# gau-nernst/llama-x

Hardware: AMD Instinct MI355X
Metric: train tokens/sec Llama-3.1-8B seq4096 at 1/2/4/8 MI355X; p50 step ms (higher is better)
Workload: dtype bf16; 1 GPU; Llama-3.1-8B text-only LoRA r=16 bf16, seq=4096, 1 sequence per GPU, causal mask, base+LM head frozen (BASELINE.json configs[1]); random-init weights at 8B dimensions; seq_len=4096, parallelism=dp1, launch=hipGraph replay (fwd+bwd+AdamW), lm_head_rows=labelled only

## Files before the change

llama-x_amd/csrc/attn_bwd.hip:

```cpp
#include "attn.h"
#include "attn_dropout.h"

typedef __attribute__((ext_vector_type(8))) short s16x8_t;

__device__ __forceinline__ int dual_swz(int row) { return ((row & 3) << 2) | ((row >> 2) & 3); }
__device__ __forceinline__ uint32_t dual_swz(uint32_t row) { return ((row & 3) << 2) | ((row >> 2) & 3); }

__device__ __forceinline__ bf16x8_t tr_frag(const char* img, int row0, int db, int lane) {
  const int hh = lane >> 5, tq = (lane & 15) >> 2, tp = lane & 3, tsub = (lane >> 4) & 1;
  const int chunk = 4 * db + 2 * tsub + (tp >> 1);
  const int rlo = row0 + 4 * hh + tq, rhi = rlo + 8;
  s16x4_t lo = __builtin_amdgcn_ds_read_tr16_b64_v4i16((lds_s16x4*)(img + rlo * 256 + ((chunk ^ dual_swz(rlo)) << 4) + ((tp & 1) << 3)));
  s16x4_t hi = __builtin_amdgcn_ds_read_tr16_b64_v4i16((lds_s16x4*)(img + rhi * 256 + ((chunk ^ dual_swz(rhi)) << 4) + ((tp & 1) << 3)));
  s16x8_t v = {lo[0], lo[1], lo[2], lo[3], hi[0], hi[1], hi[2], hi[3]};
  return __builtin_bit_cast(bf16x8_t, v);
}

__device__ __forceinline__ bf16x8_t row_frag(const char* img, int row, int ks, int hh) {
  return *reinterpret_cast<const bf16x8_t*>(img + row * 256 + (((2 * ks + hh) ^ dual_swz(row)) << 4));
}

template <int N>
__device__ __forceinline__ void lds_tr_wait(s16x4_t& a, s16x4_t& b, s16x4_t (&c)[4], s16x4_t (&d)[4]) {
  asm volatile("s_waitcnt lgkmcnt(%10)"
               : "+v"(a), "+v"(b), "+v"(c[0]), "+v"(c[1]), "+v"(c[2]), "+v"(c[3]), "+v"(d[0]), "+v"(d[1]), "+v"(d[2]), "+v"(d[3])
               : "n"(N));
  __builtin_amdgcn_sched_barrier(0);
}
__device__ __forceinline__ uint32_t xor_imm(uint32_t a, int c) {
  if (c == 0) return a;
  uint32_t r;
  asm volatile("v_xor_b32 %0, %1, %2" : "=v"(r) : "n"(c), "v"(a));
  return r;
}

struct AttnBwdArgs {
  const bf16_t* q; const bf16_t* k; const bf16_t* v; const bf16_t* o; const bf16_t* d_o;
  const float* lse; float* delta; float* nlse;
  const float* rope;
  unsigned long long* stamps;
  bf16_t* dq; bf16_t* dk; bf16_t* dv;
  bf16_t* ds; int Sp;
  int64_t q_sb, q_ss, k_sb, k_ss, v_sb, v_ss, o_sb, o_ss, do_sb, do_ss;
  int64_t dq_sb, dq_ss, dk_sb, dk_ss, dv_sb, dv_ss;
  const int* doc_ids; const int* prefix_len; const uint8_t* flags;
  int B, S, H, KVH;
  float scale, scale_log2;
  const uint8_t* mask; int64_t m_sb, m_sq;
  const int64_t* rng; uint32_t drop_thr; float drop_c; int stream_id;
};

enum { BWD_CAUSAL = 0, BWD_RULE = 1, BWD_MASK = 2 };

__device__ __forceinline__ uint32_t mask_nibble(uint32_t w) {
  const uint32_t nz = (((w & 0x7f7f7f7fu) + 0x7f7f7f7fu) | w) & 0x80808080u;
  return ((nz >> 7) * 0x01020408u) >> 24;
}

#define DQ_STAGE_BYTES (2 * TILE_BYTES)
#define DQ_LDS_BYTES (2 * DQ_STAGE_BYTES)

template <int MODE, bool DROPOUT = false>
__global__ __launch_bounds__(256, 2) void attn_bwd_dq_kernel(const AttnBwdArgs a) {
  static_assert(!(DROPOUT && MODE == BWD_MASK), "dropout exists in the causal and the rule mode");
  constexpr bool GENERAL = MODE == BWD_RULE;
  constexpr bool FLAGS = MODE != BWD_CAUSAL;
  constexpr bool MASK = MODE == BWD_MASK;
  extern __shared__ __attribute__((aligned(256))) char smem[];
  const int tid = threadIdx.x, lane = tid & 63;
  const int wave = __builtin_amdgcn_readfirstlane(tid >> 6);
  const int nqb = (a.S + BQ - 1) / BQ, nkt = (a.S + BKV - 1) / BKV;
  const int qb = nqb - 1 - blockIdx.y;
  const int h = blockIdx.x, b = blockIdx.z;
  const int kvh = h / (a.H / a.KVH);
  const int r = lane & 31, hh = lane >> 5;
  const int qi = qb * BQ + wave * 32 + r;
  const int qrow = min(qi, a.S - 1);

  const uint8_t* fl = FLAGS ? a.flags + ((int64_t)b * nqb + qb) * nkt : nullptr;
  const int kt_end = FLAGS ? nkt : min(nkt, (qb * BQ + BQ + BKV - 1) / BKV);
  uint32_t fpack = 0;
  int fchunk = -1;
  auto tile_class = [&](int t) -> int {
    if constexpr (FLAGS) {
      if ((t >> 6) != fchunk) {
        fchunk = t >> 6;
        fpack = fl[min(fchunk * 64 + lane, nkt - 1)];
      }
      return __builtin_amdgcn_readlane((int)fpack, t & 63);
    } else {
      return (t * BKV + BKV - 1 <= qb * BQ) ? 2 : 1;
    }
  };
  auto next_tile = [&](int t) {
    while (t < kt_end && tile_class(t) == 0) ++t;
    return t;
  };

  const int srow_in = lane >> 4, sslot = lane & 15;
  const bf16_t* kbase = a.k + (int64_t)b * a.k_sb + kvh * HD;
  const bf16_t* vbase = a.v + (int64_t)b * a.v_sb + kvh * HD;
  uint32_t koff[4], voff[4];
#pragma unroll
  for (int i = 0; i < 4; ++i) {
    const int row = i * 16 + wave * 4 + srow_in;
    koff[i] = (uint32_t)(((int64_t)row * a.k_ss + (sslot ^ dual_swz(row)) * 8) * 2);
    voff[i] = (uint32_t)(((int64_t)row * a.v_ss + (sslot ^ (row & 15)) * 8) * 2);
  }
  auto stage = [&](int buf, int t) {
    char* sK = smem + buf * DQ_STAGE_BYTES;
    char* sV = sK + TILE_BYTES;
    if (t * BKV + BKV <= a.S) {
      const char* kt = (const char*)(kbase + (int64_t)t * BKV * a.k_ss);
      const char* vt = (const char*)(vbase + (int64_t)t * BKV * a.v_ss);
      if constexpr (DROPOUT) {
        uint32_t l0;
        asm volatile("v_mbcnt_lo_u32_b32 %0, -1, 0\n\tv_mbcnt_hi_u32_b32 %0, -1, %0" : "=v"(l0));
        const int slot = (int)(l0 & 15);
#pragma unroll
        for (int i = 0; i < 4; ++i) {
          const int row = i * 16 + wave * 4 + (int)(l0 >> 4);
          const uint32_t ko = (uint32_t)(((int64_t)row * a.k_ss + (slot ^ dual_swz(row)) * 8) * 2);
          const uint32_t vo = (uint32_t)(((int64_t)row * a.v_ss + (slot ^ (row & 15)) * 8) * 2);
          __builtin_amdgcn_global_load_lds((gbl_void*)(kt + ko), (lds_void*)(sK + (i * 16 + wave * 4) * 256), 16, 0, 0);
          __builtin_amdgcn_global_load_lds((gbl_void*)(vt + vo), (lds_void*)(sV + (i * 16 + wave * 4) * 256), 16, 0, 0);
        }
      } else {
#pragma unroll
      for (int i = 0; i < 4; ++i) {
        __builtin_amdgcn_global_load_lds((gbl_void*)(kt + koff[i]), (lds_void*)(sK + (i * 16 + wave * 4) * 256), 16, 0, 0);
        __builtin_amdgcn_global_load_lds((gbl_void*)(vt + voff[i]), (lds_void*)(sV + (i * 16 + wave * 4) * 256), 16, 0, 0);
      }
      }
    } else {
#pragma unroll
      for (int i = 0; i < 4; ++i) {
        const int row = i * 16 + wave * 4 + srow_in;
        const int key = min(t * BKV + row, a.S - 1);
        const int kc = sslot ^ dual_swz(row);
        const int vc = sslot ^ (row & 15);
        __builtin_amdgcn_global_load_lds((gbl_void*)(kbase + (int64_t)key * a.k_ss + kc * 8), (lds_void*)(sK + (i * 16 + wave * 4) * 256), 16, 0, 0);
        __builtin_amdgcn_global_load_lds((gbl_void*)(vbase + (int64_t)key * a.v_ss + vc * 8), (lds_void*)(sV + (i * 16 + wave * 4) * 256), 16, 0, 0);
      }
// ... 15 lines not shown
  const int* docrow = (GENERAL && a.doc_ids) ? a.doc_ids + (int64_t)b * a.S : nullptr;
  const int my_doc = docrow ? docrow[qrow] : 0;
  const int my_prefix = (GENERAL && a.prefix_len) ? a.prefix_len[b] : 0;
  uint32_t mwn[MASK ? 8 : 1];
  auto mask_request = [&](int t_) {
    if constexpr (MASK) {
      uint32_t l0;
      asm volatile("v_mbcnt_lo_u32_b32 %0, -1, 0\n\tv_mbcnt_hi_u32_b32 %0, -1, %0" : "=v"(l0));
      const int hh = (int)(l0 >> 5);
      const uint8_t* mrow = a.mask + (int64_t)b * a.m_sb + (int64_t)min(qb * BQ + wave * 32 + (int)(l0 & 31), a.S - 1) * a.m_sq;
      if (t_ * BKV + BKV <= a.S) {
        const uint8_t* p = mrow + t_ * BKV + 4 * hh;
#pragma unroll
        for (int g = 0; g < 8; ++g) __builtin_memcpy(&mwn[g], p + (g >> 2) * 32 + 8 * (g & 3), 4);
      } else {
#pragma unroll
        for (int g = 0; g < 8; ++g) {
          const int g0 = t_ * BKV + (g >> 2) * 32 + 8 * (g & 3) + 4 * hh;
          __builtin_memcpy(&mwn[g], mrow + min(g0, a.S - 4), 4);
        }
      }
    }
  };
  auto mask_bits = [&](int t_) -> uint32_t {
    uint32_t bits = 0;
    if constexpr (MASK) {
      const bool ragged = t_ * BKV + BKV > a.S;
#pragma unroll
      for (int g = 0; g < 8; ++g) {
        uint32_t w = mwn[g];
        if (ragged) {
          const int g0 = t_ * BKV + (g >> 2) * 32 + 8 * (g & 3) + 4 * hh;
          const int sh = g0 - min(g0, a.S - 4);
          w = sh >= 4 ? 0u : w >> (8 * sh);
        }
        bits |= mask_nibble(w) << (4 * g);
      }
    }
    return bits;
  };

  int t = next_tile(0);
  if constexpr (MASK) {
#pragma unroll
    for (int g = 0; g < 8; ++g) mwn[g] = 0;
    if (t < kt_end && tile_class(t) == 1) mask_request(t);
  }
  if (t < kt_end) stage(0, t);
  bf16x8_t qf[8], dof[8], ovf[8];
  const float my_lse = a.lse[((int64_t)b * a.H + h) * a.S + qrow];
  {
    const bf16_t* qp = a.q + (int64_t)b * a.q_sb + (int64_t)qrow * a.q_ss + h * HD + 8 * hh;
    const bf16_t* dp = a.d_o + (int64_t)b * a.do_sb + (int64_t)qrow * a.do_ss + h * HD + 8 * hh;
    const bf16_t* op = a.o + (int64_t)b * a.o_sb + (int64_t)qrow * a.o_ss + h * HD + 8 * hh;
#pragma unroll
    for (int ks = 0; ks < 8; ++ks) {
      ovf[ks] = *reinterpret_cast<const bf16x8_t*>(op + 16 * ks);
      dof[ks] = *reinterpret_cast<const bf16x8_t*>(dp + 16 * ks);
      qf[ks] = *reinterpret_cast<const bf16x8_t*>(qp + 16 * ks);
    }
    __builtin_amdgcn_sched_barrier(0);
  }
  const float lse_safe = (my_lse == -INFINITY) ? 0.f : my_lse;
  float my_delta = 0.f;
  {
#pragma unroll
    for (int ks = 0; ks < 8; ++ks) {
#pragma unroll
      for (int j = 0; j < 8; ++j) my_delta += (float)ovf[ks][j] * (float)dof[ks][j];
    }
    my_delta += __shfl_xor(my_delta, 32, 64);
    if (hh == 0 && qi < a.S) {
      a.delta[((int64_t)b * a.H + h) * a.S + qi] = my_delta;
      a.nlse[((int64_t)b * a.H + h) * a.S + qi] = -lse_safe;
    }
  }

  asm volatile("s_waitcnt vmcnt(0)" ::: "memory");
  __syncthreads();
  int cur = 0;
  int docv = (GENERAL && docrow && t < kt_end) ? docrow[min(t * BKV + lane, a.S - 1)] : 0, docv_next = 0;
  AttnDropKey dkey = {0u, 0u};
  if constexpr (DROPOUT) dkey = attn_dropout_key(a.rng[0], a.rng[1], a.stream_id, b, h);
  while (t < kt_end) {
    int cls_m = 0;
    uint32_t mbits = 0;
    if constexpr (MASK) {
      cls_m = tile_class(t);
      if (cls_m == 1) mbits = mask_bits(t);
    }
    const int tn = next_tile(t + 1);
    if (tn < kt_end) stage(cur ^ 1, tn);
    if (GENERAL && docrow && tn < kt_end) docv_next = docrow[min(tn * BKV + lane, a.S - 1)];
    if constexpr (MASK) {
      if (tn < kt_end && tile_class(tn) == 1) mask_request(tn);
    }
    const char* sK = smem + cur * DQ_STAGE_BYTES;
    const char* sV = sK + TILE_BYTES;
    const int cls = MASK ? cls_m : tile_class(t);
#pragma unroll
    for (int kb = 0; kb < 2; ++kb) {
      f32x16_t st, dp;
      const f32x16_t zero = {0.f, 0.f, 0.f, 0.f, 0.f, 0.f, 0.f, 0.f, 0.f, 0.f, 0.f, 0.f, 0.f, 0.f, 0.f, 0.f};
      const int row = kb * 32 + r;
#pragma unroll
      for (int ks = 0; ks < 8; ++ks) {
        bf16x8_t kf = row_frag(sK, row, ks, hh);
        st = __builtin_amdgcn_mfma_f32_32x32x16_bf16(kf, qf[ks], ks == 0 ? zero : st, 0, 0, 0);
      }
      if (cls != 2) {
#pragma unroll
        for (int e = 0; e < 16; ++e) {
          if constexpr (MASK) {
            st[e] = ((mbits >> (kb * 16 + e)) & 1u) ? st[e] : -INFINITY;
          } else {
          const int kk = t * BKV + kb * 32 + (e & 3) + 8 * (e >> 2) + 4 * hh;
          bool ok = (kk < a.S) && (kk <= qi || kk < my_prefix);
          if constexpr (GENERAL) {
            const int kd = docrow ? __builtin_amdgcn_ds_bpermute((kk - t * BKV) << 2, docv) : my_doc;
            ok = ok && (kd == my_doc);
          }
          st[e] = ok ? st[e] : -INFINITY;
          }
        }
      }
#pragma unroll
      for (int e = 0; e < 16; ++e) st[e] = __builtin_amdgcn_exp2f(__builtin_fmaf(st[e], a.scale_log2, -lse_safe));
#pragma unroll
      for (int ks = 0; ks < 8; ++ks) {
        bf16x8_t vf = *reinterpret_cast<const bf16x8_t*>(sV + row * 256 + (((2 * ks + hh) ^ (row & 15)) << 4));
        dp = __builtin_amdgcn_mfma_f32_32x32x16_bf16(vf, dof[ks], ks == 0 ? zero : dp, 0, 0, 0);
      }
#pragma unroll
      for (int e = 0; e < 16; ++e) {
        float dpe = dp[e];
        if constexpr (DROPOUT) {
          const int kk = t * BKV + kb * 32 + (e & 3) + 8 * (e >> 2) + 4 * hh;
          dpe = attn_drop_keep(attn_drop_row(dkey, qi), attn_drop_col(dkey, kk), a.drop_thr) ? dpe * a.drop_c : 0.f;
        }
        st[e] = st[e] * (dpe - my_delta);
      }
      {
        const uint32_t kb_ = sbase + cur * DQ_STAGE_BYTES + kb * 8192 + aK0;
        s16x4_t Kl[4], Kh[4];
#pragma unroll
        for (int s = 0; s < 2; ++s) {
#pragma unroll
          for (int db = 0; db < 4; ++db) {
            if (s == 0) { lds_tr_read<0>(Kl[db], xor_imm(kb_, db << 6)); lds_tr_read<2048>(Kh[db], xor_imm(kb_, (db << 6) | 0x20)); }
            else { lds_tr_read<4096>(Kl[db], xor_imm(kb_, db << 6)); lds_tr_read<4096 + 2048>(Kh[db], xor_imm(kb_, (db << 6) | 0x20)); }
          }
          bf16x8_t dsb;
#pragma unroll
          for (int j = 0; j < 8; ++j) dsb[j] = (__bf16)st[8 * s + j];
          lds_tr_wait8<0>(Kl, Kh);
#pragma unroll
          for (int db = 0; db < 4; ++db) dq[db] = __builtin_amdgcn_mfma_f32_32x32x16_bf16(frag_of(Kl[db], Kh[db]), dsb, dq[db], 0, 0, 0);
          __builtin_amdgcn_sched_barrier(0);
        }
      }
    }
    asm volatile("s_waitcnt vmcnt(0)" ::: "memory");
    __syncthreads();
    cur ^= 1;
    t = tn;
    docv = docv_next;
  }

  if (qi < a.S) {
    bf16_t* op = a.dq + (int64_t)b * a.dq_sb + (int64_t)qi * a.dq_ss + h * HD;
    const bool wide = ((((uintptr_t)a.dq) | (uintptr_t)(a.dq_ss * 2) | (uintptr_t)(a.dq_sb * 2)) & 15) == 0;
#pragma unroll
    for (int db = 0; db < 4; ++db)
#pragma unroll
      for (int j2 = 0; j2 < 2; ++j2) {
        u32x2_t pp[2];
#pragma unroll
        for (int gg = 0; gg < 2; ++gg) {
          const int g4 = 2 * j2 + gg;
          u32x2_t pk;
          pk[0] = pack_bf2(dq[db][4 * g4 + 0] * a.scale, dq[db][4 * g4 + 1] * a.scale);
          pk[1] = pack_bf2(dq[db][4 * g4 + 2] * a.scale, dq[db][4 * g4 + 3] * a.scale);
          if (a.rope) {
            const f32x4_t t = *reinterpret_cast<const f32x4_t*>(a.rope + ((int64_t)qi * 64 + ((32 * db + 8 * g4 + 4 * hh) >> 1)) * 2);
            const float c0 = t[0], s0 = t[1] * -1.f, c1 = t[2], s1 = t[3] * -1.f;
            const float x0 = bflo(pk[0]), x1 = bfhi(pk[0]), y0 = bflo(pk[1]), y1 = bfhi(pk[1]);
            pk[0] = pack_bf2(x0 * c0 - x1 * s0, x1 * c0 + x0 * s0);
            pk[1] = pack_bf2(y0 * c1 - y1 * s1, y1 * c1 + y0 * s1);
          }
          pp[gg] = pk;
        }
        if (wide) {
          const auto r0 = __builtin_amdgcn_permlane32_swap(pp[0][0], pp[1][0], false, false);
          const auto r1 = __builtin_amdgcn_permlane32_swap(pp[0][1], pp[1][1], false, false);
          *reinterpret_cast<u32x4_t*>(op + 32 * db + 16 * j2 + 8 * hh) = u32x4_t{r0[0], r1[0], r0[1], r1[1]};
        } else {
          *reinterpret_cast<u32x2_t*>(op + 32 * db + 16 * j2 + 4 * hh) = pp[0];
          *reinterpret_cast<u32x2_t*>(op + 32 * db + 16 * j2 + 8 + 4 * hh) = pp[1];
        }
      }
  }
}

#define DKV_QT 64
#define DKV2_KEYS 128

typedef __attribute__((address_space(3))) char lds_char;
typedef __attribute__((address_space(3))) bf16x8_t lds_bf16x8;
typedef __attribute__((address_space(3))) f32x4_t lds_f32x4;
#define DKV3_LDS_BYTES (0x10000 + 1024)

template <int MODE, bool STAMP = false, bool DS = false, bool DROPOUT = false>
__global__ __launch_bounds__(256, 2) void attn_bwd_dkv3_kernel(const AttnBwdArgs a, float* __restrict__ part) {
  static_assert(!(DROPOUT && (MODE == BWD_MASK || STAMP || DS)), "dropout exists on the default route, in the causal and the rule mode");
  constexpr bool GENERAL = MODE == BWD_RULE;
  constexpr bool FLAGS = MODE != BWD_CAUSAL;
  constexpr bool MASK = MODE == BWD_MASK;
  static_assert(!(MASK && (STAMP || DS)), "the dense-mask mode exists on the default route only");
  extern __shared__ __attribute__((aligned(256))) char smem[];
  const int tid = threadIdx.x, lane = tid & 63;
  const int wave = __builtin_amdgcn_readfirstlane(tid >> 6);
  const int nqb = (a.S + BQ - 1) / BQ, nkt = (a.S + BKV - 1) / BKV;
  const int nqt = (a.S + DKV_QT - 1) / DKV_QT;
  const int G = a.H / a.KVH;
  int id = blockIdx.x;
  const int per_kb = a.B * a.KVH * G;
  const int kblk = id / per_kb;
  id -= kblk * per_kb;
  const int b = id / (a.KVH * G);
  id -= b * (a.KVH * G);
  const int kvh = id / G, g = id % G;
  const int h = kvh * G + g;
  const int my_kt = 2 * kblk + (wave >> 1);

  bf16x8_t kf[8], vf[8];
  const int* docrow = (GENERAL && a.doc_ids) ? a.doc_ids + (int64_t)b * a.S : nullptr;
  int key_doc = 0;
  {
    const int krow = min(kblk * DKV2_KEYS + wave * 32 + (lane & 31), a.S - 1);
    const bf16_t* kp = a.k + (int64_t)b * a.k_sb + (int64_t)krow * a.k_ss + kvh * HD + 8 * (lane >> 5);
    const bf16_t* vp = a.v + (int64_t)b * a.v_sb + (int64_t)krow * a.v_ss + kvh * HD + 8 * (lane >> 5);
#pragma unroll
    for (int ks = 0; ks < 8; ++ks) {
      kf[ks] = *reinterpret_cast<const bf16x8_t*>(kp + 16 * ks);
      vf[ks] = *reinterpret_cast<const bf16x8_t*>(vp + 16 * ks);
    }
    if (docrow) key_doc = docrow[krow];
  }
  const int my_prefix = (GENERAL && a.prefix_len) ? a.prefix_len[b] : 0;

  const int qt_first = FLAGS ? 0 : (kblk * DKV2_KEYS) / DKV_QT;
  uint32_t fpack = 0;
  int fchunk = -1;
  auto block_class = [&](int qt, int kt) -> int {
    if (kt >= nkt) return 0;
    if constexpr (FLAGS) {
      const int qb128 = qt >> 1;
      if ((qb128 >> 6) != fchunk) {
        fchunk = qb128 >> 6;
        uint32_t ln;
        asm volatile("v_mbcnt_lo_u32_b32 %0, -1, 0\n\tv_mbcnt_hi_u32_b32 %0, -1, %0" : "=v"(ln));
        const uint8_t* fr = a.flags + ((int64_t)b * nqb + min(fchunk * 64 + (int)ln, nqb - 1)) * nkt;
        fpack = (uint32_t)fr[2 * kblk] | ((2 * kblk + 1 < nkt ? (uint32_t)fr[2 * kblk + 1] : 0u) << 8);
      }
      const uint32_t w = (uint32_t)__builtin_amdgcn_readlane((int)fpack, qb128 & 63);
      return (int)((w >> (8 * (kt - 2 * kblk))) & 0xff);
    }
    const int q_lo = qt * DKV_QT, q_hi = q_lo + DKV_QT - 1, k_lo = kt * BKV, k_hi = k_lo + BKV - 1;
    if (k_lo > q_hi) return 0;
    return (k_hi <= q_lo) ? 2 : 1;
  };
  auto next_qt = [&](int qt) {
    while (qt < nqt && !(qt >= qt_first && (block_class(qt, 2 * kblk) != 0 || block_class(qt, 2 * kblk + 1) != 0))) ++qt;
    return qt;
  };

  const uint32_t sbase = (uint32_t)(uintptr_t)(lds_char*)smem;

  const char* qbase = (const char*)(a.q + (int64_t)b * a.q_sb + h * HD);
  const char* dbase = (const char*)(a.d_o + (int64_t)b * a.do_sb + h * HD);
  const float* lbase = (wave == 0 ? a.nlse : a.delta) + ((int64_t)b * a.H + h) * a.S;
  auto stage = [&](int buf, int qt) {
    uint32_t ln;
    asm volatile("v_mbcnt_lo_u32_b32 %0, -1, 0\n\tv_mbcnt_hi_u32_b32 %0, -1, %0" : "=v"(ln));
    const uint32_t srow = wave * 4 + (ln >> 4);
    const uint32_t sc = (ln & 15) ^ dual_swz(srow);
    lds_char* sQ = (lds_char*)smem + buf * 0x8000 + wave * 1024;
    if (qt * DKV_QT + DKV_QT <= a.S) {
      const uint32_t q_lane = (srow * (uint32_t)a.q_ss + sc * 8) * 2, d_lane = (srow * (uint32_t)a.do_ss + sc * 8) * 2;
#pragma unroll
      for (int i = 0; i < 4; ++i) {
        const char* qu = qbase + (int64_t)(qt * DKV_QT + i * 16) * a.q_ss * 2;
        const char* du = dbase + (int64_t)(qt * DKV_QT + i * 16) * a.do_ss * 2;
        __builtin_amdgcn_global_load_lds((gbl_void*)(qu + q_lane), (lds_void*)(sQ + i * 4096), 16, 0, 0);
        __builtin_amdgcn_global_load_lds((gbl_void*)(du + d_lane), (lds_void*)(sQ + 0x4000 + i * 4096), 16, 0, 0);
      }
    } else {
#pragma unroll
      for (int i = 0; i < 4; ++i) {
        const int qr = min(qt * DKV_QT + i * 16 + (int)srow, a.S - 1);
        __builtin_amdgcn_global_load_lds((gbl_void*)(qbase + ((int64_t)qr * a.q_ss + sc * 8) * 2), (lds_void*)(sQ + i * 4096), 16, 0, 0);
// ... 11 lines not shown
  for (int i = 0; i < 4; ++i)
#pragma unroll
    for (int e = 0; e < 16; ++e) { dk[i][e] = 0.f; dv[i][e] = 0.f; }

  uint32_t mwn[MASK ? 8 : 1];
  auto mask_request = [&](int qt_) {
    if constexpr (MASK) {
      uint32_t l0;
      asm volatile("v_mbcnt_lo_u32_b32 %0, -1, 0\n\tv_mbcnt_hi_u32_b32 %0, -1, %0" : "=v"(l0));
      const uint8_t* mr = a.mask + (int64_t)b * a.m_sb + (int64_t)min(qt_ * DKV_QT + (int)l0, a.S - 1) * a.m_sq;
      const int key0 = kblk * DKV2_KEYS + wave * 32;
      if (key0 + 32 <= a.S) {
#pragma unroll
        for (int g = 0; g < 8; ++g) __builtin_memcpy(&mwn[g], mr + key0 + 4 * g, 4);
      } else {
#pragma unroll
        for (int g = 0; g < 8; ++g) __builtin_memcpy(&mwn[g], mr + min(key0 + 4 * g, a.S - 4), 4);
      }
    }
  };
  auto mask_bits = [&]() -> uint32_t {
    uint32_t bits = 0;
    if constexpr (MASK) {
#pragma unroll
      for (int g = 0; g < 8; ++g) asm volatile("" : "+v"(mwn[g]));
      const bool ragged = kblk * DKV2_KEYS + wave * 32 + 32 > a.S;
#pragma unroll
      for (int g = 0; g < 8; ++g) {
        uint32_t w = mwn[g];
        if (ragged) {
          const int g0 = kblk * DKV2_KEYS + wave * 32 + 4 * g;
          const int sh = g0 - min(g0, a.S - 4);
          w = sh >= 4 ? 0u : w >> (8 * sh);
        }
        bits |= mask_nibble(w) << (4 * g);
      }
    }
    return bits;
  };

  auto mask_wanted = [&](int qt_) -> bool {
    const int c = block_class(qt_, my_kt);
    return c == 1 || (c == 2 && qt_ * DKV_QT + DKV_QT > a.S);
  };
  int qt = next_qt(0);
  if constexpr (MASK) {
#pragma unroll
    for (int g = 0; g < 8; ++g) mwn[g] = 0;
    if (qt < nqt && mask_wanted(qt)) mask_request(qt);
  }
  int qdoc = 0, qdoc_next = 0;
  if (GENERAL && docrow && qt < nqt) {
    uint32_t l0;
    asm volatile("v_mbcnt_lo_u32_b32 %0, -1, 0\n\tv_mbcnt_hi_u32_b32 %0, -1, %0" : "=v"(l0));
    qdoc = docrow[min(qt * DKV_QT + (int)l0, a.S - 1)];
  }
  if (qt < nqt) stage(0, qt);
  asm volatile("s_waitcnt vmcnt(0)" ::: "memory");
  __syncthreads();
  int cur = 0;
  AttnDropKey dkey = {0u, 0u};
  if constexpr (DROPOUT) dkey = attn_dropout_key(a.rng[0], a.rng[1], a.stream_id, b, h);
  int nst = 0;
  auto stamp = [&]() {
    if constexpr (STAMP) {
      if (blockIdx.x == 0 && wave == 0 && nst < 1024) {
        unsigned long long tt;
        asm volatile("s_memtime %0\n\ts_waitcnt lgkmcnt(0)" : "=s"(tt) :: "memory");
        if (threadIdx.x == 0) a.stamps[nst] = tt;
        ++nst;
      }
    }
  };
  while (qt < nqt) {
    stamp();
    const int qtn = next_qt(qt + 1);
    const bool have_next = qtn < nqt;
    uint32_t ln;
    asm volatile("v_mbcnt_lo_u32_b32 %0, -1, 0\n\tv_mbcnt_hi_u32_b32 %0, -1, %0" : "=v"(ln));
    const uint32_t lr_ = ln & 31, lh_ = ln >> 5;
    const uint32_t Lr = sbase + cur * 0x8000 + lr_ * 256 + ((lh_ ^ dual_swz(lr_)) << 4);
    const uint32_t tq = (ln & 15) >> 2, tp = ln & 3, tsub = (ln >> 4) & 1, trow = 4 * lh_ + tq;
    const uint32_t Tl = sbase + cur * 0x8000 + trow * 256 + (((2 * tsub + (tp >> 1)) ^ dual_swz(trow)) << 4) + ((tp & 1) << 3);
    const uint32_t Th = sbase + cur * 0x8000 + (trow + 8) * 256 + (((2 * tsub + (tp >> 1)) ^ dual_swz(trow + 8)) << 4) + ((tp & 1) << 3);
    const uint32_t Ls = sbase + 0x10000 + cur * 512 + lh_ * 16;
    const int hh = (int)lh_;
    const int key = kblk * DKV2_KEYS + wave * 32 + (int)lr_;
    int cls = block_class(qt, my_kt);
    if (cls == 2 && (qt * DKV_QT + DKV_QT > a.S)) cls = 1;
    uint32_t rowbits = 0;
    if constexpr (MASK) {
      if (cls == 1) rowbits = mask_bits();
      __builtin_amdgcn_sched_barrier(0);
    }
    if (have_next) stage(cur ^ 1, qtn);
    if (GENERAL && docrow && have_next) qdoc_next = docrow[min(qtn * DKV_QT + (int)ln, a.S - 1)];
    stamp();
    if (cls != 0) {
      auto rowf = [&](int qb32, int img, int ks) -> bf16x8_t {
        return *(lds_bf16x8*)((lds_char*)(uintptr_t)xor_imm(Lr, ks << 5) + qb32 * 8192 + img * 0x4000);
      };
      auto trf = [&](int qb32, int img, int step, s16x4_t& tl, s16x4_t& th) {
        const int s2 = step >> 2, db = step & 3;
        lds_tr_read_rt(tl, xor_imm(Tl, db << 6), (qb32 * 32 + s2 * 16) * 256 + img * 0x4000);
        lds_tr_read_rt(th, xor_imm(Th, db << 6), (qb32 * 32 + s2 * 16) * 256 + img * 0x4000);
      };
#pragma unroll
      for (int qb32 = 0; qb32 < 2; ++qb32) {
        f32x16_t st, dp;
        const f32x16_t zero = {0.f, 0.f, 0.f, 0.f, 0.f, 0.f, 0.f, 0.f, 0.f, 0.f, 0.f, 0.f, 0.f, 0.f, 0.f, 0.f};
        bf16x8_t f3[3];
        f3[0] = rowf(qb32, 0, 0);
        f3[1] = rowf(qb32, 0, 1);
#pragma unroll
        for (int ks = 0; ks < 8; ++ks) {
          if (ks + 2 < 8) f3[(ks + 2) % 3] = rowf(qb32, 0, ks + 2);
          st = __builtin_amdgcn_mfma_f32_32x32x16_bf16(f3[ks % 3], kf[ks], ks == 0 ? zero : st, 0, 0, 0);
          __builtin_amdgcn_sched_barrier(0);
        }
        if (qb32 == 0) stamp();
        bf16x8_t g3[3];
        g3[0] = rowf(qb32, 1, 0);
        g3[1] = rowf(qb32, 1, 1);
        if (cls != 2) {
#pragma unroll
          for (int e = 0; e < 16; ++e) {
            const int qi = qt * DKV_QT + qb32 * 32 + 8 * (e >> 2) + 4 * hh + (e & 3);
            if constexpr (MASK) {
              const uint32_t rb = (uint32_t)__builtin_amdgcn_ds_bpermute((qi - qt * DKV_QT) << 2, (int)rowbits);
              st[e] = ((qi < a.S) && ((rb >> lr_) & 1u)) ? st[e] : -INFINITY;
            } else {
            bool ok = (qi < a.S) && (key < a.S) && (key <= qi || key < my_prefix);
            if constexpr (GENERAL) {
              const int qd = docrow ? __builtin_amdgcn_ds_bpermute((qi - qt * DKV_QT) << 2, qdoc) : key_doc;
              ok = ok && (qd == key_doc);
            }
            st[e] = ok ? st[e] : -INFINITY;
            }
          }
        }
#pragma unroll
        for (int g4 = 0; g4 < 4; ++g4) {
          const f32x4_t l4 = *(lds_f32x4*)((lds_char*)(uintptr_t)Ls + (qb32 * 32 + 8 * g4) * 4);
#pragma unroll
          for (int e2 = 0; e2 < 4; ++e2) st[4 * g4 + e2] = __builtin_amdgcn_exp2f(__builtin_fmaf(st[4 * g4 + e2], a.scale_log2, l4[e2]));
        }
        __builtin_amdgcn_sched_barrier(0);
        if (qb32 == 0) stamp();
#pragma unroll
        for (int ks = 0; ks < 8; ++ks) {
          if (ks + 2 < 8) g3[(ks + 2) % 3] = rowf(qb32, 1, ks + 2);
          dp = __builtin_amdgcn_mfma_f32_32x32x16_bf16(g3[ks % 3], vf[ks], ks == 0 ? zero : dp, 0, 0, 0);
          __builtin_amdgcn_sched_barrier(0);
        }
        if (qb32 == 0) stamp();
        s16x4_t tdl[2], tdh[2], tql[2], tqh[2];
        if constexpr (!DROPOUT) {
          trf(qb32, 1, 0, tdl[0], tdh[0]);
          trf(qb32, 0, 0, tql[0], tqh[0]);
        }
        bf16x8_t pb[2], dsb[2];
#pragma unroll
        for (int g4 = 0; g4 < 4; ++g4) {
          const f32x4_t d4 = *(lds_f32x4*)((lds_char*)(uintptr_t)Ls + 256 + (qb32 * 32 + 8 * g4) * 4);
#pragma unroll
          for (int e2 = 0; e2 < 4; ++e2) {
            const int e = 4 * g4 + e2;
            if constexpr (DROPOUT) {
              const int qi = qt * DKV_QT + qb32 * 32 + 8 * g4 + 4 * hh + e2;
              const bool keep = attn_drop_keep(attn_drop_row(dkey, qi), attn_drop_col(dkey, key), a.drop_thr);
              pb[e >> 3][e & 7] = (__bf16)(keep ? st[e] * a.drop_c : 0.f);
              dsb[e >> 3][e & 7] = (__bf16)(st[e] * ((keep ? dp[e] * a.drop_c : 0.f) - d4[e2]));
            } else {
            pb[e >> 3][e & 7] = (__bf16)st[e];
            dsb[e >> 3][e & 7] = (__bf16)(st[e] * (dp[e] - d4[e2]));
            }
          }
        }
        if constexpr (DS) {
          bf16_t* dtile = a.ds + ((int64_t)b * a.H + h) * a.Sp * a.Sp + (int64_t)(my_kt * (a.Sp >> 7) + (qt >> 1)) * (64 * 128);
#pragma unroll
          for (int s2 = 0; s2 < 2; ++s2) {
            const u32x4_t w = __builtin_bit_cast(u32x4_t, dsb[s2]);
            const auto r0 = __builtin_amdgcn_permlane32_swap(w[0], w[2], false, false);
            const auto r1 = __builtin_amdgcn_permlane32_swap(w[1], w[3], false, false);
            const int piece = ((((wave & 1) * 2 + (qt & 1)) * 2 + qb32) * 2 + s2) * 64;
            *reinterpret_cast<u32x4_t*>(dtile + (piece + (int)ln) * 8) = u32x4_t{r0[0], r1[0], r0[1], r1[1]};
          }
        }
        if constexpr (DROPOUT) {
          __builtin_amdgcn_sched_barrier(0);
          trf(qb32, 1, 0, tdl[0], tdh[0]);
          trf(qb32, 0, 0, tql[0], tqh[0]);
        }
        __builtin_amdgcn_sched_barrier(0);
        if (qb32 == 0) stamp();
#pragma unroll
        for (int step = 0; step < 8; ++step) {
          if (step + 1 < 8) {
            trf(qb32, 1, step + 1, tdl[(step + 1) & 1], tdh[(step + 1) & 1]);
            trf(qb32, 0, step + 1, tql[(step + 1) & 1], tqh[(step + 1) & 1]);
          }
          if (step + 1 < 8) lds_tr_wait4<4>(tdl[step & 1], tdh[step & 1], tql[step & 1], tqh[step & 1]);
          else lds_tr_wait4<0>(tdl[step & 1], tdh[step & 1], tql[step & 1], tqh[step & 1]);
          dv[step & 3] = __builtin_amdgcn_mfma_f32_32x32x16_bf16(frag_of(tdl[step & 1], tdh[step & 1]), pb[step >> 2], dv[step & 3], 0, 0, 0);
          dk[step & 3] = __builtin_amdgcn_mfma_f32_32x32x16_bf16(frag_of(tql[step & 1], tqh[step & 1]), dsb[step >> 2], dk[step & 3], 0, 0, 0);
          __builtin_amdgcn_sched_barrier(0);
        }
        if (qb32 == 0) stamp();
      }
    }
    if constexpr (MASK) {
#pragma unroll
      for (int g = 0; g < 8; ++g) mwn[g] = 0;
      if (have_next && mask_wanted(qtn)) mask_request(qtn);
    }
    stamp();
    asm volatile("s_waitcnt vmcnt(0)" ::: "memory");
    stamp();
    __syncthreads();
    stamp();
    cur ^= 1;
    qt = qtn;
    qdoc = qdoc_next;
  }

  const int64_t plane = (int64_t)a.B * a.S * a.KVH * HD;
  uint32_t le;
  asm volatile("v_mbcnt_lo_u32_b32 %0, -1, 0\n\tv_mbcnt_hi_u32_b32 %0, -1, %0" : "=v"(le));
  const int hh = (int)(le >> 5);
  const int key = kblk * DKV2_KEYS + wave * 32 + (int)(le & 31);
  if (key < a.S) {
    float* pk = part + (int64_t)(g * 2 + 0) * plane + (((int64_t)b * a.S + key) * a.KVH + kvh) * HD;
    float* pv = part + (int64_t)(g * 2 + 1) * plane + (((int64_t)b * a.S + key) * a.KVH + kvh) * HD;
#pragma unroll
    for (int db = 0; db < 4; ++db)
#pragma unroll
      for (int g4 = 0; g4 < 4; ++g4) {
        const int d = 32 * db + 8 * g4 + 4 * hh;
        *reinterpret_cast<f32x4_t*>(pk + d) = f32x4_t{dk[db][4 * g4], dk[db][4 * g4 + 1], dk[db][4 * g4 + 2], dk[db][4 * g4 + 3]};
        *reinterpret_cast<f32x4_t*>(pv + d) = f32x4_t{dv[db][4 * g4], dv[db][4 * g4 + 1], dv[db][4 * g4 + 2], dv[db][4 * g4 + 3]};
      }
  }
}

__global__ __launch_bounds__(256) void attn_bwd_delta_kernel(const AttnBwdArgs a) {
  const int64_t idx = (int64_t)blockIdx.x * 16 + (threadIdx.x >> 4);
  const int c = threadIdx.x & 15;
  const int64_t total = (int64_t)a.B * a.S * a.H;
  const int64_t i = idx < total ? idx : total - 1;
  const int h = (int)(i % a.H);
  const int64_t bq = i / a.H;
  const int q = (int)(bq % a.S), b = (int)(bq / a.S);
  const u32x4_t ov = *reinterpret_cast<const u32x4_t*>(a.o + (int64_t)b * a.o_sb + (int64_t)q * a.o_ss + h * HD + c * 8);
  const u32x4_t dv = *reinterpret_cast<const u32x4_t*>(a.d_o + (int64_t)b * a.do_sb + (int64_t)q * a.do_ss + h * HD + c * 8);
  float s = 0.f;
#pragma unroll
  for (int e = 0; e < 4; ++e) s += bflo(ov[e]) * bflo(dv[e]) + bfhi(ov[e]) * bfhi(dv[e]);
  s += __shfl_xor(s, 1, 64);
  s += __shfl_xor(s, 2, 64);
  s += __shfl_xor(s, 4, 64);
  s += __shfl_xor(s, 8, 64);
  if (c == 0 && idx < total) {
    const int64_t o = ((int64_t)b * a.H + h) * a.S + q;
    const float l = a.lse[o];
    a.delta[o] = s;
    a.nlse[o] = (l == -INFINITY) ? 0.f : -l;
  }
}

#define DQ2_BQ 256
#define DQ2_STAGE_BYTES (3 * TILE_BYTES)
#define DQ2_STAGES 3
#define DQ2_LDS_BYTES (DQ2_STAGES * DQ2_STAGE_BYTES)

template <bool GENERAL>
__global__ __launch_bounds__(512, 2) void attn_bwd_dq2_kernel(const AttnBwdArgs a) {
  extern __shared__ __attribute__((aligned(256))) char smem[];
  const int tid = threadIdx.x, lane = tid & 63;
  const int wave = __builtin_amdgcn_readfirstlane(tid >> 6);
  const int nqb = (a.S + BQ - 1) / BQ, nkt = (a.S + BKV - 1) / BKV;
  const int nqb2 = (a.S + DQ2_BQ - 1) / DQ2_BQ;
  const int qb2 = nqb2 - 1 - blockIdx.y;
  const int h = blockIdx.x, b = blockIdx.z;
  const int kvh = h / (a.H / a.KVH);
  const int r = lane & 31, hh = lane >> 5;
// ... 344 lines not shown
```

llama-x_amd/csrc/common.h:

```cpp
#pragma once
#include <hip/hip_runtime.h>
#include <stdint.h>
#include <stdarg.h>
#include <stdio.h>

#define LLX_OK 0
#define LLX_ERR_ARG -1
#define LLX_ERR_LAUNCH -2
#define LLX_ERR_UNSUPPORTED -3

void llx_set_error(const char* fmt, ...);

#define LLX_REQUIRE(cond, ...)            \
  do {                                    \
    if (!(cond)) {                        \
      llx_set_error(__VA_ARGS__);         \
      return LLX_ERR_ARG;                 \
    }                                     \
  } while (0)

#define LLX_LAUNCH_CHECK(name)                                              \
  do {                                                                      \
    hipError_t e__ = hipGetLastError();                                     \
    if (e__ != hipSuccess) {                                                \
// ... 105 lines not shown
  for (int e = 0; e < 4; ++e) {
    float dgs[2], dus[2];
#pragma unroll
    for (int p = 0; p < 2; ++p) {
      const float gg = p ? bfhi(gv[e]) : bflo(gv[e]);
      const float uu = p ? bfhi(uv[e]) : bflo(uv[e]);
      const float dd = p ? bfhi(dv[e]) : bflo(dv[e]);
      const float sg = sigmoidf_(gg);
      const float silu = bf2f(f2bf(gg * sg));
      dus[p] = dd * silu;
      const float ds = bf2f(f2bf(dd * uu));
      dgs[p] = ds * (sg * (1.f + gg * (1.f - sg)));
    }
    og[e] = pack_bf2(dgs[0], dgs[1]);
    ou[e] = pack_bf2(dus[0], dus[1]);
  }
}

__device__ __forceinline__ u32x4_t rope8(const u32x4_t& v, const f32x4_t& t0, const f32x4_t& t1, float sign) {
  const float cs[4] = {t0[0], t0[2], t1[0], t1[2]};
  const float sn[4] = {t0[1] * sign, t0[3] * sign, t1[1] * sign, t1[3] * sign};
  u32x4_t o;
#pragma unroll
  for (int e = 0; e < 4; ++e) {
    const float x0 = bflo(v[e]), x1 = bfhi(v[e]);
    o[e] = pack_bf2(x0 * cs[e] - x1 * sn[e], x1 * cs[e] + x0 * sn[e]);
  }
  return o;
}

__device__ __forceinline__ u32x4_t rope8(const u32x4_t& v, const float* __restrict__ tp, float sign) {
  const f32x4_t t0 = *reinterpret_cast<const f32x4_t*>(tp);
  const f32x4_t t1 = *reinterpret_cast<const f32x4_t*>(tp + 4);
  const float cs[4] = {t0[0], t0[2], t1[0], t1[2]};
  const float sn[4] = {t0[1] * sign, t0[3] * sign, t1[1] * sign, t1[3] * sign};
  u32x4_t o;
#pragma unroll
  for (int e = 0; e < 4; ++e) {
    const float x0 = bflo(v[e]), x1 = bfhi(v[e]);
    o[e] = pack_bf2(x0 * cs[e] - x1 * sn[e], x1 * cs[e] + x0 * sn[e]);
  }
  return o;
}

typedef __attribute__((ext_vector_type(8))) short llx_s16x8_t;
template <int OFF>
__device__ __forceinline__ void lds_tr_read(s16x4_t& dst, uint32_t addr) {
  asm volatile("ds_read_b64_tr_b16 %0, %1 offset:%2" : "=v"(dst) : "v"(addr), "n"(OFF));
}
__device__ __forceinline__ void lds_tr_read_rt(s16x4_t& dst, uint32_t addr, int off) {
  asm volatile("ds_read_b64_tr_b16 %0, %1 offset:%2" : "=v"(dst) : "v"(addr), "n"(off));
}
template <int N>
__device__ __forceinline__ void lds_tr_wait4(s16x4_t& a, s16x4_t& b, s16x4_t& c, s16x4_t& d) {
  asm volatile("s_waitcnt lgkmcnt(%4)" : "+v"(a), "+v"(b), "+v"(c), "+v"(d) : "n"(N));
  __builtin_amdgcn_sched_barrier(0);
}
template <int N>
__device__ __forceinline__ void lds_tr_wait8(s16x4_t (&c)[4], s16x4_t (&d)[4]) {
  asm volatile("s_waitcnt lgkmcnt(%8)" : "+v"(c[0]), "+v"(c[1]), "+v"(c[2]), "+v"(c[3]), "+v"(d[0]), "+v"(d[1]), "+v"(d[2]), "+v"(d[3]) : "n"(N));
  __builtin_amdgcn_sched_barrier(0);
}
__device__ __forceinline__ void lds_read16_rt(i32x4_t& dst, uint32_t addr, int off) {
  asm volatile("ds_read_b128 %0, %1 offset:%2" : "=v"(dst) : "v"(addr), "n"(off));
}
template <typename T>
__device__ __forceinline__ void lds_pin1(T& x) { asm volatile("" : "+v"(x)); }
template <typename T, int N>
__device__ __forceinline__ void lds_pin1(T (&x)[N]) {
#pragma unroll
  for (int i = 0; i < N; ++i) asm volatile("" : "+v"(x[i]));
}
template <typename... T>
__device__ __forceinline__ void lds_pin(T&... x) {
  (lds_pin1(x), ...);
  __builtin_amdgcn_sched_barrier(0);
}
template <int N, typename... T>
__device__ __forceinline__ void lds_wait(T&... x) {
  asm volatile("s_waitcnt lgkmcnt(%0)" : : "n"(N));
  (lds_pin1(x), ...);
  __builtin_amdgcn_sched_barrier(0);
}
__device__ __forceinline__ bf16x8_t frag_of(const s16x4_t& lo, const s16x4_t& hi) {
  const llx_s16x8_t v = {lo[0], lo[1], lo[2], lo[3], hi[0], hi[1], hi[2], hi[3]};
  return __builtin_bit_cast(bf16x8_t, v);
}

typedef __attribute__((address_space(3))) void llx_lds_void;
__device__ __forceinline__ __amdgpu_buffer_rsrc_t lds_dma_rsrc(const void* base, uint32_t bytes) {
  return __builtin_amdgcn_make_buffer_rsrc(const_cast<void*>(base), 0, (int)bytes, 0x00020000);
}
__device__ __forceinline__ void lds_dma16(__amdgpu_buffer_rsrc_t rsrc, llx_lds_void* dst, uint32_t lane_off, uint32_t wave_off) {
  __builtin_amdgcn_raw_ptr_buffer_load_lds(rsrc, dst, 16, (int)lane_off, (int)wave_off, 0, 0);
}
```

Before: 32160 tokens/s.

## Software-pipeline LDS fragment reads with explicit lgkmcnt waits in attention backward kernels

Rewrites the inner loops of the dQ and causal dK/dV backward kernels so LDS row fragments, LSE/delta stats, and transposed K reads are issued ahead through inline asm into a three-slot ring. Each MFMA then waits on an exact lgkmcnt count instead of relying on compiler scheduling. The exp2 work is interleaved with the dP MFMAs, and the first fragments of the next sub-block are prefetched early. This aims to hide LDS latency behind matrix ops, at the cost of fragile hand-computed wait counts and higher register pressure.

Result: no change. 32190 tokens/s, median of 6 (+0.1%).

```diff
diff --git a/llama-x_amd/csrc/attn_bwd.hip b/llama-x_amd/csrc/attn_bwd.hip
--- a/llama-x_amd/csrc/attn_bwd.hip
+++ b/llama-x_amd/csrc/attn_bwd.hip
@@ -59,6 +59,16 @@
 
 #define DQ_STAGE_BYTES (2 * TILE_BYTES)
 #define DQ_LDS_BYTES (2 * DQ_STAGE_BYTES)
+
+#define DQ_TR_LEAD 4
+constexpr int dq_frag_wait(int i) {
+  int n = 0;
+  for (int j = i - 2; j <= i; ++j) {
+    if (j > i - 2 && j + 2 < 16) ++n;
+    if (j >= 16 - DQ_TR_LEAD) n += 2;
+  }
+  return n;
+}
 
 template <int MODE, bool DROPOUT = false>
 __global__ __launch_bounds__(256, 2) void attn_bwd_dq_kernel(const AttnBwdArgs a) {
@@ -240,7 +250,16 @@
   int docv = (GENERAL && docrow && t < kt_end) ? docrow[min(t * BKV + lane, a.S - 1)] : 0, docv_next = 0;
   AttnDropKey dkey = {0u, 0u};
   if constexpr (DROPOUT) dkey = attn_dropout_key(a.rng[0], a.rng[1], a.stream_id, b, h);
+  const uint32_t LK = sbase + r * 256 + ((hh ^ dual_swz(r)) << 4);
+  const uint32_t LV = sbase + TILE_BYTES + r * 256 + ((hh ^ (r & 15)) << 4);
   while (t < kt_end) {
+    const uint32_t Kc = LK + cur * DQ_STAGE_BYTES, Vc = LV + cur * DQ_STAGE_BYTES;
+    i32x4_t fr[3];
+    auto frag_read = [&](int kb, int i) {
+      if (i < 16) lds_read16_rt(fr[i % 3], xor_imm(i < 8 ? Kc : Vc, (i & 7) << 5), kb * 8192);
+    };
+    frag_read(0, 0);
+    frag_read(0, 1);
     int cls_m = 0;
     uint32_t mbits = 0;
     if constexpr (MASK) {
@@ -253,18 +272,19 @@
     if constexpr (MASK) {
       if (tn < kt_end && tile_class(tn) == 1) mask_request(tn);
     }
-    const char* sK = smem + cur * DQ_STAGE_BYTES;
-    const char* sV = sK + TILE_BYTES;
     const int cls = MASK ? cls_m : tile_class(t);
 #pragma unroll
     for (int kb = 0; kb < 2; ++kb) {
       f32x16_t st, dp;
       const f32x16_t zero = {0.f, 0.f, 0.f, 0.f, 0.f, 0.f, 0.f, 0.f, 0.f, 0.f, 0.f, 0.f, 0.f, 0.f, 0.f, 0.f};
-      const int row = kb * 32 + r;
-#pragma unroll
-      for (int ks = 0; ks < 8; ++ks) {
-        bf16x8_t kf = row_frag(sK, row, ks, hh);
-        st = __builtin_amdgcn_mfma_f32_32x32x16_bf16(kf, qf[ks], ks == 0 ? zero : st, 0, 0, 0);
+      const uint32_t kb_ = sbase + cur * DQ_STAGE_BYTES + kb * 8192 + aK0;
+      s16x4_t Kl[2][4], Kh[2][4];
+#pragma unroll
+      for (int i = 0; i < 8; ++i) {
+        frag_read(kb, i + 2);
+        if (i == 0) lds_wait<2>(fr[0]);
+        else lds_wait<2>(fr[i % 3], st);
+        st = __builtin_amdgcn_mfma_f32_32x32x16_bf16(__builtin_bit_cast(bf16x8_t, fr[i % 3]), qf[i], i == 0 ? zero : st, 0, 0, 0);
       }
       if (cls != 2) {
 #pragma unroll
@@ -283,12 +303,29 @@
         }
       }
 #pragma unroll
-      for (int e = 0; e < 16; ++e) st[e] = __builtin_amdgcn_exp2f(__builtin_fmaf(st[e], a.scale_log2, -lse_safe));
-#pragma unroll
-      for (int ks = 0; ks < 8; ++ks) {
-        bf16x8_t vf = *reinterpret_cast<const bf16x8_t*>(sV + row * 256 + (((2 * ks + hh) ^ (row & 15)) << 4));
-        dp = __builtin_amdgcn_mfma_f32_32x32x16_bf16(vf, dof[ks], ks == 0 ? zero : dp, 0, 0, 0);
-      }
+      for (int i = 8; i < 16; ++i) {
+        if (i + 2 < 16) frag_read(kb, i + 2);
+        if (i >= 16 - DQ_TR_LEAD) {
+          const int db = i - (16 - DQ_TR_LEAD);
+          lds_tr_read<0>(Kl[0][db], xor_imm(kb_, db << 6));
+          lds_tr_read<2048>(Kh[0][db], xor_imm(kb_, (db << 6) | 0x20));
+        }
+        if (i == 8) lds_wait_rt(dq_frag_wait(8), fr[8 % 3], st);
+        else lds_wait_rt(dq_frag_wait(i), fr[i % 3], dp);
+        dp = __builtin_amdgcn_mfma_f32_32x32x16_bf16(__builtin_bit_cast(bf16x8_t, fr[i % 3]), dof[i - 8], i == 8 ? zero : dp, 0, 0, 0);
+#pragma unroll
+        for (int e = 2 * (i - 8); e < 2 * (i - 8) + 2; ++e) st[e] = __builtin_amdgcn_exp2f(__builtin_fmaf(st[e], a.scale_log2, -lse_safe));
+      }
+#pragma unroll
+      for (int s = 0; s < 2; ++s) {
+#pragma unroll
+        for (int db = (s == 0 ? DQ_TR_LEAD : 0); db < 4; ++db) {
+          if (s == 0) { lds_tr_read<0>(Kl[0][db], xor_imm(kb_, db << 6)); lds_tr_read<2048>(Kh[0][db], xor_imm(kb_, (db << 6) | 0x20)); }
+          else { lds_tr_read<4096>(Kl[1][db], xor_imm(kb_, db << 6)); lds_tr_read<4096 + 2048>(Kh[1][db], xor_imm(kb_, (db << 6) | 0x20)); }
+        }
+      }
+      if (kb == 0) { frag_read(1, 0); frag_read(1, 1); }
+      __builtin_amdgcn_sched_barrier(0);
 #pragma unroll
       for (int e = 0; e < 16; ++e) {
         float dpe = dp[e];
@@ -298,24 +335,18 @@
         }
         st[e] = st[e] * (dpe - my_delta);
       }
-      {
-        const uint32_t kb_ = sbase + cur * DQ_STAGE_BYTES + kb * 8192 + aK0;
-        s16x4_t Kl[4], Kh[4];
-#pragma unroll
-        for (int s = 0; s < 2; ++s) {
-#pragma unroll
-          for (int db = 0; db < 4; ++db) {
-            if (s == 0) { lds_tr_read<0>(Kl[db], xor_imm(kb_, db << 6)); lds_tr_read<2048>(Kh[db], xor_imm(kb_, (db << 6) | 0x20)); }
-            else { lds_tr_read<4096>(Kl[db], xor_imm(kb_, db << 6)); lds_tr_read<4096 + 2048>(Kh[db], xor_imm(kb_, (db << 6) | 0x20)); }
-          }
-          bf16x8_t dsb;
-#pragma unroll
-          for (int j = 0; j < 8; ++j) dsb[j] = (__bf16)st[8 * s + j];
-          lds_tr_wait8<0>(Kl, Kh);
-#pragma unroll
-          for (int db = 0; db < 4; ++db) dq[db] = __builtin_amdgcn_mfma_f32_32x32x16_bf16(frag_of(Kl[db], Kh[db]), dsb, dq[db], 0, 0, 0);
-          __builtin_amdgcn_sched_barrier(0);
-        }
+#pragma unroll
+      for (int s = 0; s < 2; ++s) {
+        bf16x8_t dsb;
+#pragma unroll
+        for (int j = 0; j < 8; ++j) dsb[j] = (__bf16)st[8 * s + j];
+        if (s == 0 && kb == 0) lds_tr_wait8<10>(Kl[0], Kh[0]);
+        else if (s == 0) lds_tr_wait8<8>(Kl[0], Kh[0]);
+        else if (kb == 0) lds_tr_wait8<2>(Kl[1], Kh[1]);
+        else lds_tr_wait8<0>(Kl[1], Kh[1]);
+#pragma unroll
+        for (int db = 0; db < 4; ++db) dq[db] = __builtin_amdgcn_mfma_f32_32x32x16_bf16(frag_of(Kl[s][db], Kh[s][db]), dsb, dq[db], 0, 0, 0);
+        __builtin_amdgcn_sched_barrier(0);
       }
     }
     asm volatile("s_waitcnt vmcnt(0)" ::: "memory");
@@ -368,6 +399,16 @@
 typedef __attribute__((address_space(3))) f32x4_t lds_f32x4;
 #define DKV3_LDS_BYTES (0x10000 + 1024)
 
+constexpr int dkv_slot_pre(int j) { return j == 7 ? 2 : (j == 14 || j == 15) ? 1 : 0; }
+constexpr int dkv_slot_post(int j) { return j == 7 ? 2 : 0; }
+constexpr int dkv_frag_wait(int i) {
+  int n = i >= 2 ? dkv_slot_pre(i - 2) + dkv_slot_post(i - 2) : 0;
+  if (i >= 1) n += dkv_slot_pre(i - 1) + dkv_slot_post(i - 1);
+  n += dkv_slot_pre(i);
+  for (int j = i - 1; j <= i; ++j) n += j + 2 < 16 ? 1 : 0;
+  return n;
+}
+
 template <int MODE, bool STAMP = false, bool DS = false, bool DROPOUT = false>
 __global__ __launch_bounds__(256, 2) void attn_bwd_dkv3_kernel(const AttnBwdArgs a, float* __restrict__ part) {
   static_assert(!(DROPOUT && (MODE == BWD_MASK || STAMP || DS)), "dropout exists on the default route, in the causal and the rule mode");
@@ -375,6 +416,7 @@
   constexpr bool FLAGS = MODE != BWD_CAUSAL;
   constexpr bool MASK = MODE == BWD_MASK;
   static_assert(!(MASK && (STAMP || DS)), "the dense-mask mode exists on the default route only");
+  constexpr bool RING = MODE == BWD_CAUSAL;
   extern __shared__ __attribute__((aligned(256))) char smem[];
   const int tid = threadIdx.x, lane = tid & 63;
   const int wave = __builtin_amdgcn_readfirstlane(tid >> 6);
@@ -552,7 +594,6 @@
     const uint32_t Lr = sbase + cur * 0x8000 + lr_ * 256 + ((lh_ ^ dual_swz(lr_)) << 4);
     const uint32_t tq = (ln & 15) >> 2, tp = ln & 3, tsub = (ln >> 4) & 1, trow = 4 * lh_ + tq;
     const uint32_t Tl = sbase + cur * 0x8000 + trow * 256 + (((2 * tsub + (tp >> 1)) ^ dual_swz(trow)) << 4) + ((tp & 1) << 3);
-    const uint32_t Th = sbase + cur * 0x8000 + (trow + 8) * 256 + (((2 * tsub + (tp >> 1)) ^ dual_swz(trow + 8)) << 4) + ((tp & 1) << 3);
     const uint32_t Ls = sbase + 0x10000 + cur * 512 + lh_ * 16;
     const int hh = (int)lh_;
     const int key = kblk * DKV2_KEYS + wave * 32 + (int)lr_;
@@ -567,31 +608,56 @@
     if (GENERAL && docrow && have_next) qdoc_next = docrow[min(qtn * DKV_QT + (int)ln, a.S - 1)];
     stamp();
     if (cls != 0) {
+      auto trf = [&](int qb32, int img, int step, s16x4_t& tl, s16x4_t& th) {
+        const int s2 = step >> 2, db = step & 3;
+        lds_tr_read_rt(tl, xor_imm(Tl, db << 6), (qb32 * 32 + s2 * 16) * 256 + img * 0x4000);
+        lds_tr_read_rt(th, xor_imm(Tl, (db << 6) | 0x20), (qb32 * 32 + s2 * 16 + 8) * 256 + img * 0x4000);
+      };
+      i32x4_t fr[3];
+      auto row_read = [&](int qb32, int i) {
+        if (i < 16) lds_read16_rt(fr[i % 3], xor_imm(Lr, (i & 7) << 5), qb32 * 8192 + (i < 8 ? 0 : 0x4000));
+      };
+      auto stat_read = [&](i32x4_t& dst, int qb32, int which, int g4) {
+        lds_read16_rt(dst, Ls, which * 256 + (qb32 * 32 + 8 * g4) * 4);
+      };
       auto rowf = [&](int qb32, int img, int ks) -> bf16x8_t {
         return *(lds_bf16x8*)((lds_char*)(uintptr_t)xor_imm(Lr, ks << 5) + qb32 * 8192 + img * 0x4000);
       };
-      auto trf = [&](int qb32, int img, int step, s16x4_t& tl, s16x4_t& th) {
-        const int s2 = step >> 2, db = step & 3;
-        lds_tr_read_rt(tl, xor_imm(Tl, db << 6), (qb32 * 32 + s2 * 16) * 256 + img * 0x4000);
-        lds_tr_read_rt(th, xor_imm(Th, db << 6), (qb32 * 32 + s2 * 16) * 256 + img * 0x4000);
-      };
 #pragma unroll
       for (int qb32 = 0; qb32 < 2; ++qb32) {
         f32x16_t st, dp;
         const f32x16_t zero = {0.f, 0.f, 0.f, 0.f, 0.f, 0.f, 0.f, 0.f, 0.f, 0.f, 0.f, 0.f, 0.f, 0.f, 0.f, 0.f};
-        bf16x8_t f3[3];
-        f3[0] = rowf(qb32, 0, 0);
-        f3[1] = rowf(qb32, 0, 1);
-#pragma unroll
-        for (int ks = 0; ks < 8; ++ks) {
-          if (ks + 2 < 8) f3[(ks + 2) % 3] = rowf(qb32, 0, ks + 2);
-          st = __builtin_amdgcn_mfma_f32_32x32x16_bf16(f3[ks % 3], kf[ks], ks == 0 ? zero : st, 0, 0, 0);
-          __builtin_amdgcn_sched_barrier(0);
+        i32x4_t sl[4], sd[4];
+        bf16x8_t g3[3];
+        if constexpr (RING) {
+          if (qb32 == 0) { row_read(0, 0); row_read(0, 1); }
+#pragma unroll
+          for (int i = 0; i < 8; ++i) {
+            row_read(qb32, i + 2);
+            if (i == 7) { stat_read(sl[0], qb32, 0, 0); stat_read(sl[1], qb32, 0, 1); }
+            if (i == 0) lds_wait_rt(dkv_frag_wait(0), fr[0]);
+            else lds_wait_rt(dkv_frag_wait(i), fr[i % 3], st);
+            st = __builtin_amdgcn_mfma_f32_32x32x16_bf16(__builtin_bit_cast(bf16x8_t, fr[i % 3]), kf[i], i == 0 ? zero : st, 0, 0, 0);
+            __builtin_amdgcn_sched_barrier(0);
+          }
+          stat_read(sl[2], qb32, 0, 2);
+          stat_read(sl[3], qb32, 0, 3);
+        } else {
+          bf16x8_t f3[3];
+          f3[0] = rowf(qb32, 0, 0);
+          f3[1] = rowf(qb32, 0, 1);
+#pragma unroll
+          for (int ks = 0; ks < 8; ++ks) {
+            if (ks + 2 < 8) f3[(ks + 2) % 3] = rowf(qb32, 0, ks + 2);
+            st = __builtin_amdgcn_mfma_f32_32x32x16_bf16(f3[ks % 3], kf[ks], ks == 0 ? zero : st, 0, 0, 0);
+            __builtin_amdgcn_sched_barrier(0);
+          }
         }
         if (qb32 == 0) stamp();
-        bf16x8_t g3[3];
-        g3[0] = rowf(qb32, 1, 0);
-        g3[1] = rowf(qb32, 1, 1);
+        if constexpr (!RING) {
+          g3[0] = rowf(qb32, 1, 0);
+          g3[1] = rowf(qb32, 1, 1);
+        }
         if (cls != 2) {
 #pragma unroll
           for (int e = 0; e < 16; ++e) {
@@ -609,30 +675,63 @@
             }
           }
         }
+        if constexpr (RING) lds_wait<2>(sl[0], sl[1]);
 #pragma unroll
         for (int g4 = 0; g4 < 4; ++g4) {
-          const f32x4_t l4 = *(lds_f32x4*)((lds_char*)(uintptr_t)Ls + (qb32 * 32 + 8 * g4) * 4);
+          if constexpr (RING) {
+            if (g4 == 2) lds_wait<0>(sl[2], sl[3]);
+          }
+          f32x4_t l4;
+          if constexpr (RING) l4 = __builtin_bit_cast(f32x4_t, sl[g4]);
+          else l4 = *(lds_f32x4*)((lds_char*)(uintptr_t)Ls + (qb32 * 32 + 8 * g4) * 4);
 #pragma unroll
           for (int e2 = 0; e2 < 4; ++e2) st[4 * g4 + e2] = __builtin_amdgcn_exp2f(__builtin_fmaf(st[4 * g4 + e2], a.scale_log2, l4[e2]));
         }
         __builtin_amdgcn_sched_barrier(0);
         if (qb32 == 0) stamp();
-#pragma unroll
-        for (int ks = 0; ks < 8; ++ks) {
-          if (ks + 2 < 8) g3[(ks + 2) % 3] = rowf(qb32, 1, ks + 2);
-          dp = __builtin_amdgcn_mfma_f32_32x32x16_bf16(g3[ks % 3], vf[ks], ks == 0 ? zero : dp, 0, 0, 0);
-          __builtin_amdgcn_sched_barrier(0);
-        }
-        if (qb32 == 0) stamp();
         s16x4_t tdl[2], tdh[2], tql[2], tqh[2];
+        if constexpr (RING) {
+#pragma unroll
+          for (int i = 8; i < 16; ++i) {
+            row_read(qb32, i + 2);
+            if (i == 14) stat_read(sd[0], qb32, 1, 0);
+            if (i == 15) stat_read(sd[1], qb32, 1, 1);
+            if (i == 8) lds_wait_rt(dkv_frag_wait(8), fr[8 % 3]);
+            else lds_wait_rt(dkv_frag_wait(i), fr[i % 3], dp);
+            dp = __builtin_amdgcn_mfma_f32_32x32x16_bf16(__builtin_bit_cast(bf16x8_t, fr[i % 3]), vf[i - 8], i == 8 ? zero : dp, 0, 0, 0);
+            __builtin_amdgcn_sched_barrier(0);
+          }
+        } else {
+#pragma unroll
+          for (int ks = 0; ks < 8; ++ks) {
+            if (ks + 2 < 8) g3[(ks + 2) % 3] = rowf(qb32, 1, ks + 2);
+            dp = __builtin_amdgcn_mfma_f32_32x32x16_bf16(g3[ks % 3], vf[ks], ks == 0 ? zero : dp, 0, 0, 0);
+            __builtin_amdgcn_sched_barrier(0);
+          }
+        }
         if constexpr (!DROPOUT) {
           trf(qb32, 1, 0, tdl[0], tdh[0]);
           trf(qb32, 0, 0, tql[0], tqh[0]);
         }
+        if (qb32 == 0) stamp();
+        if constexpr (RING) lds_wait<DROPOUT ? 0 : 4>(sd[0], sd[1], dp);
         bf16x8_t pb[2], dsb[2];
 #pragma unroll
         for (int g4 = 0; g4 < 4; ++g4) {
-          const f32x4_t d4 = *(lds_f32x4*)((lds_char*)(uintptr_t)Ls + 256 + (qb32 * 32 + 8 * g4) * 4);
+          f32x4_t d4;
+          if constexpr (RING) {
+            if (g4 == 1) { lds_pin(pb[0], dsb[0]); stat_read(sd[2], qb32, 1, 2); }
+            if (g4 == 2) {
+              lds_pin(pb[0], dsb[0]);
+              stat_read(sd[3], qb32, 1, 3);
+              if constexpr (DROPOUT) lds_wait<1>(sd[2]);
+              else lds_wait<1>(sd[2], tdl[0], tdh[0], tql[0], tqh[0]);
+            }
+            if (g4 == 3) lds_wait<0>(sd[3]);
+            d4 = __builtin_bit_cast(f32x4_t, sd[g4]);
+          } else {
+            d4 = *(lds_f32x4*)((lds_char*)(uintptr_t)Ls + 256 + (qb32 * 32 + 8 * g4) * 4);
+          }
 #pragma unroll
           for (int e2 = 0; e2 < 4; ++e2) {
             const int e = 4 * g4 + e2;
@@ -671,7 +770,9 @@
             trf(qb32, 1, step + 1, tdl[(step + 1) & 1], tdh[(step + 1) & 1]);
             trf(qb32, 0, step + 1, tql[(step + 1) & 1], tqh[(step + 1) & 1]);
           }
+          if (RING && step == 7 && qb32 == 0) { row_read(1, 0); row_read(1, 1); }
           if (step + 1 < 8) lds_tr_wait4<4>(tdl[step & 1], tdh[step & 1], tql[step & 1], tqh[step & 1]);
+          else if (RING && qb32 == 0) lds_tr_wait4<2>(tdl[step & 1], tdh[step & 1], tql[step & 1], tqh[step & 1]);
           else lds_tr_wait4<0>(tdl[step & 1], tdh[step & 1], tql[step & 1], tqh[step & 1]);
           dv[step & 3] = __builtin_amdgcn_mfma_f32_32x32x16_bf16(frag_of(tdl[step & 1], tdh[step & 1]), pb[step >> 2], dv[step & 3], 0, 0, 0);
           dk[step & 3] = __builtin_amdgcn_mfma_f32_32x32x16_bf16(frag_of(tql[step & 1], tqh[step & 1]), dsb[step >> 2], dk[step & 3], 0, 0, 0);
diff --git a/llama-x_amd/csrc/common.h b/llama-x_amd/csrc/common.h
--- a/llama-x_amd/csrc/common.h
+++ b/llama-x_amd/csrc/common.h
@@ -211,6 +211,12 @@
   (lds_pin1(x), ...);
   __builtin_amdgcn_sched_barrier(0);
 }
+template <typename... T>
+__device__ __forceinline__ void lds_wait_rt(int n, T&... x) {
+  asm volatile("s_waitcnt lgkmcnt(%0)" : : "n"(n));
+  (lds_pin1(x), ...);
+  __builtin_amdgcn_sched_barrier(0);
+}
 __device__ __forceinline__ bf16x8_t frag_of(const s16x4_t& lo, const s16x4_t& hi) {
   const llx_s16x8_t v = {lo[0], lo[1], lo[2], lo[3], hi[0], hi[1], hi[2], hi[3]};
   return __builtin_bit_cast(bf16x8_t, v);
```
